# MPI-SWS/RedQueen

Measured on AMD Instinct MI355X. Metric: redqueen_replicas_per_sec, higher is better.
Workload: dtype f64; 1 GPU; C3 syn1k: 1000 followers, 50 sources (25 Poisson2 rate 1 + 25 Hawkes l0=1 a=1 b=10), degree 5, T=100, q=1e6, s=1, RedQueen, randomized worlds; replicas_per_gpu=10000, global_batch=10000, parallelism=replica-sharded dp1, replicas_per_chunk=10000

## Files before the change

redqueen_amd/csrc/rq_api.cpp:

```cpp
#include <hip/hip_runtime.h>

#include <algorithm>
#include <cstring>
#include <memory>
#include <mutex>
#include <new>
#include <vector>

#include "../../include/rq.h"
#include "rq_internal.h"

using rqh::align_up;
using rqh::CtrlTables;
using rqh::GraphTopo;
using rqh::Knobs;
using rqh::Plan;

namespace {

template <class T>
struct DevBuf {
    T* p = nullptr;
    size_t n = 0;
    ~DevBuf() { if (p) (void)hipFree(p); }
// ... 537 lines not shown

int rq_graph_source_ids(rq_graph_t g, int64_t* ids)
{
    if (!g || !ids) return RQ_EINVAL;
    std::copy(g->src_id.begin(), g->src_id.end(), ids);
    return RQ_OK;
}

int rq_graph_followers(rq_graph_t g, int64_t* ids)
{
    if (!g || !ids) return RQ_EINVAL;
    std::copy(g->fol_ids.begin(), g->fol_ids.end(), ids);
    return RQ_OK;
}

int rq_workspace_size(rq_graph_t g, const rq_batch_desc* b, size_t* bytes)
{
    if (!bytes) return RQ_EINVAL;
    Plan p;
    const int rc = plan_call(g, b, rqh::read_knobs(), 0.0, &p);
    if (rc) return rc;
    *bytes = p.total;
    return RQ_OK;
}

int rq_plan_info(rq_graph_t g, const rq_batch_desc* b, int64_t* info)
{
    return rq_plan_info_n(g, b, info, 8);
}

int rq_plan_info_n(rq_graph_t g, const rq_batch_desc* b, int64_t* out, int n)
{
    if (!out || n < 0) return RQ_EINVAL;
    int64_t info[9];
    Plan p;
    const int rc = plan_call(g, b, rqh::read_knobs(), 0.0, &p);
    if (rc) return rc;
    rqh::plan_info(p, b->ctrl_kind, info);
    std::copy(info, info + std::min(n, 9), out);
    return RQ_OK;
}

int rq_event_capacity(rq_graph_t g, const rq_batch_desc* b, int64_t* cap)
{
    if (!cap) return RQ_EINVAL;
    Plan p;
    const int rc = plan_call(g, b, rqh::read_knobs(), 0.0, &p);
    if (rc) return rc;
    *cap = p.cap_rows;
    return RQ_OK;
}

int rq_run_batch(rq_graph_t g, const rq_batch_desc* b, const rq_outputs* out, void* workspace,
                 size_t workspace_bytes, void* hip_stream)
{
    const Knobs kn = rqh::read_knobs();
    Plan p;
    int rc = plan_call(g, b, kn, (double)workspace_bytes, &p);
    if (rc) return rc;
    if (!out || !out->metrics || !out->counts || !out->status || !workspace) return RQ_EINVAL;
    if (workspace_bytes < p.total) return RQ_EINVAL;
    if ((b->flags & RQ_RUN_EVENT_LOG) && (!out->ev_t || !out->ev_src || out->ev_cap < 1))
        return RQ_EINVAL;
    char* ws = (char*)workspace;
    hipStream_t pst[3] = {(hipStream_t)hip_stream, nullptr, nullptr};

    if ((rc = stage_tables(g, p, b, rqh::ctrl_tables(*g, b), ws, pst[0]))) return rc;
    if (hipMemsetAsync(out->status, 0, sizeof(int32_t) * p.R, pst[0]) != hipSuccess) return RQ_EHIP;
    Join join{pst, t_pipes.of(pst[0])};
    if ((rc = fork_streams(p.nbuf, &join))) return rc;

    int64_t ci = 0;
// ... 501 lines not shown
```

redqueen_amd/csrc/rq_device.h:

```cpp
#pragma once
#include <hip/hip_runtime.h>
#include <stdint.h>

#include "rq_spec.h"

#pragma clang fp contract(off)

#define RQ_INF __builtin_huge_val()

namespace rq {

static __constant__ uint64_t rq_exp_tab_c[RQ_EXP_TAB_N] = RQ_EXP_TAB_INIT;

__device__ __forceinline__ void philox4x32_10(uint32_t c[4], uint32_t k0, uint32_t k1)
{
#pragma unroll
    for (int r = 0; r < 10; ++r) {
        const uint64_t p0 = (uint64_t)0xD2511F53u * c[0];
        const uint64_t p1 = (uint64_t)0xCD9E8D57u * c[2];
        const uint32_t n0 = (uint32_t)(p1 >> 32) ^ c[1] ^ k0;
        const uint32_t n2 = (uint32_t)(p0 >> 32) ^ c[3] ^ k1;
        c[0] = n0;
        c[1] = (uint32_t)p1;
        c[2] = n2;
// ... 44 lines not shown
}

__device__ __forceinline__ double wave_min(double v)
{
#pragma unroll
    for (int o = 32; o > 0; o >>= 1) v = fmin(v, __shfl_xor(v, o, 64));
    return v;
}

__device__ __forceinline__ double bcast_d(double v, int src_lane)
{
    const uint64_t b = rq_dbl_bits(v);
    const uint32_t lo = (uint32_t)__builtin_amdgcn_readlane((int)(uint32_t)b, src_lane);
    const uint32_t hi = (uint32_t)__builtin_amdgcn_readlane((int)(uint32_t)(b >> 32), src_lane);
    return rq_bits_dbl(((uint64_t)hi << 32) | lo);
}

__device__ __forceinline__ int bcast_i(int v, int src_lane)
{
    return __builtin_amdgcn_readlane(v, src_lane);
}

__device__ __forceinline__ uint64_t sgpr_u64(uint64_t v)
{
    const uint32_t lo = (uint32_t)__builtin_amdgcn_readfirstlane((int)(uint32_t)v);
    const uint32_t hi = (uint32_t)__builtin_amdgcn_readfirstlane((int)(uint32_t)(v >> 32));
    return ((uint64_t)hi << 32) | lo;
}
__device__ __forceinline__ int64_t bcast_i64(int64_t v, int src_lane)
{
    const uint32_t lo = (uint32_t)__builtin_amdgcn_readlane((int)(uint32_t)v, src_lane);
    const uint32_t hi = (uint32_t)__builtin_amdgcn_readlane((int)(uint32_t)((uint64_t)v >> 32), src_lane);
    return (int64_t)(((uint64_t)hi << 32) | lo);
}

__device__ __forceinline__ void wave_lds_sync()
{
    __builtin_amdgcn_fence(__ATOMIC_RELEASE, "wavefront");
    __builtin_amdgcn_wave_barrier();
    __builtin_amdgcn_fence(__ATOMIC_ACQUIRE, "wavefront");
}
__device__ __forceinline__ void wave_mem_sync()
{
    __builtin_amdgcn_fence(__ATOMIC_RELEASE, "workgroup");
    __builtin_amdgcn_wave_barrier();
    __builtin_amdgcn_fence(__ATOMIC_ACQUIRE, "workgroup");
}

__device__ __forceinline__ int popc(uint64_t m) { return __popcll(m); }

template <int CTRL, int ROWMASK>
__device__ __forceinline__ uint32_t dpp_u32(uint32_t v)
{
    return (uint32_t)__builtin_amdgcn_update_dpp((int)0xFFFFFFFF, (int)v, CTRL, ROWMASK, 0xF, false);
}
__device__ __forceinline__ uint32_t umin32(uint32_t a, uint32_t b) { return a < b ? a : b; }

__device__ __forceinline__ uint32_t wave_min_u32(uint32_t v)
{
    v = umin32(v, dpp_u32<0xB1, 0xF>(v));
    v = umin32(v, dpp_u32<0x4E, 0xF>(v));
    v = umin32(v, dpp_u32<0x141, 0xF>(v));
    v = umin32(v, dpp_u32<0x140, 0xF>(v));
    v = umin32(v, dpp_u32<0x142, 0xA>(v));
    v = umin32(v, dpp_u32<0x143, 0xC>(v));
    return (uint32_t)__builtin_amdgcn_readlane((int)v, 63);
// ... 87 lines not shown
        v |= dpp0<0x111, 0xF>(v) & c0;
        v |= dpp0<0x112, 0xF>(v) & c1;
        v |= dpp0<0x114, 0xF>(v) & c2;
        v |= dpp0<0x118, 0xF>(v) & c3;
        v |= dpp0<0x142, 0xA>(v) & c4;
        v |= dpp0<0x143, 0xC>(v) & c5;
        return v;
    }
    __device__ __forceinline__ uint32_t scan_or_z(uint32_t m) const
    {
        uint32_t t = dppz<0x111>(m);
        uint32_t v = m | (t & c0);
        t = dppz<0x112>(v);
        v |= t & c1;
        t = dppz<0x114>(v);
        v |= t & c2;
        t = dppz<0x118>(v);
        v |= t & c3;
        t = (uint32_t)__builtin_amdgcn_update_dpp((int)t, (int)v, 0x142, 0xA, 0xF, false);
        v |= t & c4;
        t = (uint32_t)__builtin_amdgcn_update_dpp((int)t, (int)v, 0x143, 0xC, 0xF, false);
        v |= t & c5;
        return v;
    }
    __device__ __forceinline__ uint32_t scan_add(uint32_t v) const
    {
        v += dpp0<0x111, 0xF>(v) & c0;
        v += dpp0<0x112, 0xF>(v) & c1;
        v += dpp0<0x114, 0xF>(v) & c2;
        v += dpp0<0x118, 0xF>(v) & c3;
        v += dpp0<0x142, 0xA>(v) & c4;
        v += dpp0<0x143, 0xC>(v) & c5;
        return v;
    }
};

__device__ __forceinline__ int stage_rank(const double* st_t, int n, double ti, int lane)
{
    int rnk = 0;
    for (int q = 0; q < n; q += 8) {
        double2 x[4];
#pragma unroll
        for (int u = 0; u < 4; ++u) x[u] = *reinterpret_cast<const double2*>(st_t + q + 2 * u);
#pragma unroll
        for (int u = 0; u < 4; ++u) rnk += (x[u].x < ti ? 1 : 0) + (x[u].y < ti ? 1 : 0);
    }
    const uint32_t sum = wave_sum_u32(lane < n ? (uint32_t)rnk : 0u);
    if (sum == (uint32_t)(n * (n - 1) / 2)) return rnk;
    rnk = 0;
    for (int q = 0; q < n; q += 2) {
        const double2 x = *reinterpret_cast<const double2*>(st_t + q);
        rnk += (x.x < ti || (x.x == ti && q < lane)) ? 1 : 0;
        rnk += (x.y < ti || (x.y == ti && q + 1 < lane)) ? 1 : 0;
    }
    return rnk;
}

__device__ __forceinline__ double min_raw(double a, double b)
{
    double r;
    __asm__("v_min_f64 %0, %1, %2\n\ts_nop 1" : "=v"(r) : "v"(a), "v"(b));
    return r;
}

__device__ __forceinline__ double wave_min_f64(double x)
{
// ... 340 lines not shown
```

redqueen_amd/csrc/rq_host.h:

```cpp
#pragma once
#include <stddef.h>
#include <stdint.h>

#include <vector>

#include "../../include/rq.h"

#define RQ_MAX_STREAMS 2048
#define RQ_NPSUM1_LDS 516
#ifndef RQ_MRG_LB
#define RQ_MRG_LB 1024
#endif
#define RQ_MG_B 512
#define RQ_MAX_STREAMS_MRG (RQ_MG_B * RQ_MG_B)

struct SweepInst {
    bool fused;
    int nK;
    bool col16;
    bool log;
    bool gs;
    bool bits;
    bool bl;
    bool mrg;
    int spl;
    int W;
    bool gt;
    bool pw;
    bool pair;
    bool scan;
};
#define RQ_FWS_NL 66
#define RQ_FWS_LDS_BYTES(nK) ((size_t)8 * (((nK) + 2 + 3) * RQ_FWS_NL + 4))

#ifndef RQ_FOLLOWERS_TILE_SINKS
#define RQ_FOLLOWERS_TILE_SINKS 2048
#endif
static_assert(RQ_FOLLOWERS_TILE_SINKS >= 1 &&
                  (long long)RQ_FOLLOWERS_TILE_SINKS * (12 + 8 * (RQ_MAX_K + 2) + 8) <= 160 * 1024,
              "a tile of every nK / rows variant must fit one workgroup's LDS");

int rq_sweep_blocks_per_cu(const SweepInst& i, int wpb, size_t lds);
int rq_fw_blocks_per_cu(const SweepInst& i, int wpb, size_t lds);
int rq_cu_count();

namespace rqh {

inline size_t align_up(size_t x, size_t a) { return (x + a - 1) / a * a; }

inline int followers_tiles(int n_sinks) { return (n_sinks + RQ_FOLLOWERS_TILE_SINKS - 1) / RQ_FOLLOWERS_TILE_SINKS; }
inline size_t followers_tiled_ws_bytes(int n_sinks, int64_t n_rep)
{
    return align_up((size_t)4 * (size_t)n_rep * (size_t)followers_tiles(n_sinks), 256);
}

template <class T>
struct Knob {
    bool set = false;
    T v{};
};
struct Knobs {
    Knob<double> ws_budget_gb;
    double cap_squeeze = 1.0;
    Knob<int> mg_grp;
    bool mrg = true;
    Knob<int> g_collds;
    int g_w = 0;
    bool skip = true;
    bool fwm = true;
    bool ctrl_draws = true;
    bool sweep_scan = true;
    int fw_w = 0;
    int pipe = 2;
    Knob<int64_t> pipe_chunk;
    bool order = false;

    int sweep_dbg = 0;
    double fw_tile = 58.0;
    Knob<int> fw_hmin, fw_thr, fw_hfill;
    int fw_static = 0;
    bool clk_merge = false;

    Knob<int> rp_chunk;
    bool rp_small = true;
    bool clk_replay = false;
};
Knobs read_knobs();

struct GraphTopo {
    int n_str = 0, ctrl_idx = -1, n_sinks = 0, n_fol = 0;
    int64_t n_edges = 0, ctrl_src_id = 0;
    double start = 0.0, end = 0.0;
    std::vector<int64_t> src_id;
    std::vector<int> kind, orig_idx, arr_off, arr_n;
    std::vector<int> is_static;
    std::vector<uint32_t> seed;
    std::vector<double> p0, p1, p2, arr_a, arr_b;
    std::vector<int> csr_ptr, csr_col, outdeg_f, fol;
    std::vector<int64_t> fol_ids;
    std::vector<int64_t> sink_ids;
    std::vector<int> csr_col_el;
    std::vector<int> col_to_fol;
    bool multi = false, ctrl_dup = false;
    bool rd_ties = false, rd_ties_ctrl = false;
// ... 5 lines not shown
    int n_tiles = 0;
    std::vector<int> tile_ptr, tile_col;
    int ctrl_arr_off = 0, ctrl_arr_n = 0;
};
int topo_build(const rq_graph_desc* d, GraphTopo* g);

struct Plan {
    int nK = 1, spl = 1, wpb = 4, n_sinks_pad = 0;
    int64_t R = 0, chunk = 0, capsum = 0, cap_rows = 0;
    int64_t rep_lo = 0, rep_cnt = 0;
    std::vector<int> cap;
    std::vector<int64_t> st_off;
    std::vector<int> rd_k;
    bool log = false, bits = false;
    bool bl = false;
    size_t g_fb = 0, g_etab = 0, g_inv = 0, g_skip = 0;
    bool g_inv_sh = false;
    bool gs = false;
    int64_t gs_slots = 0, gs_stride = 0;
    bool fw = false;
    int fw_h = 8, mstride = 1;
    bool mrg = false;
    bool lmrg = false;
    bool gt = false;
    size_t off_mt = 0, off_mj = 0, off_mjh = 0, off_mlen = 0;
    int64_t mrg_stride = 0;
    int n_grp = 1;
    int grp_sz = RQ_MG_B;
    int64_t sub_stride = 0;
    size_t off_sub_t = 0, off_sub_j = 0, off_sub_len = 0;
    bool fwm = false;
    bool pair = false;
    bool scan = false;
    int gwpb = 4, gwin = 16, gcol_lds = 1, gcol16 = 0;
    size_t g_col = 0, g_ptr = 0, g_odf = 0, g_cbf = 0, g_wave = 0, g_wave_stride = 0, g_rank_off = 0,
           g_win_off = 0, g_x_off = 0, g_total = 0, g_stage_off = 0;
    size_t tables_bytes = 0;
    int wpc = 0;
    int nbuf = 1;
    bool order = false;
    size_t off_set0 = 0, set_stride = 0, off_ord = 0;
    size_t off_pwc = 0, off_pwmax = 0;
    size_t off_invc = 0, off_streams = 0, off_slen = 0, off_rt = 0, off_rs = 0, off_rv = 0,
           off_rc = 0, off_sall = 0, off_wq = 0, off_stoff = 0, off_cap = 0, off_rdk = 0, off_repidx = 0, off_gs = 0,
           total = 0;
};

int make_plan(const GraphTopo& g, const rq_batch_desc* b, const Knobs& kn, double budget, Plan* p);
SweepInst sweep_inst(const Plan& p, int ctrl_kind);
void plan_info(const Plan& p, int ctrl_kind, int64_t info[9]);

struct CtrlTables {
    std::vector<double> invc;
    std::vector<double> pwc, pwmax;
};
CtrlTables ctrl_tables(const GraphTopo& g, const rq_batch_desc* b);

}
```

redqueen_amd/csrc/rq_plan.cpp:

```cpp
#include <algorithm>
#include <cmath>
#include <cstdlib>

#include "rq_host.h"
#include "rq_tables.h"

namespace rqh {

Knobs read_knobs()
{
    Knobs k;
    if (const char* e = getenv("RQ_WS_BUDGET_GB")) k.ws_budget_gb = {true, atof(e)};
    if (const char* e = getenv("RQ_CAP_SQUEEZE")) k.cap_squeeze = std::max(0.01, std::min(1.0, atof(e)));
    if (const char* e = getenv("RQ_MG_GRP")) k.mg_grp = {true, atoi(e)};
    if (const char* e = getenv("RQ_MRG")) k.mrg = atoi(e) != 0;
    if (const char* e = getenv("RQ_G_COLLDS")) k.g_collds = {true, atoi(e)};
    if (const char* e = getenv("RQ_G_W")) k.g_w = atoi(e);
    if (const char* e = getenv("RQ_SKIP")) k.skip = atoi(e) != 0;
    if (const char* e = getenv("RQ_FWM")) k.fwm = atoi(e) != 0;
    if (const char* e = getenv("RQ_CTRL_DRAWS")) k.ctrl_draws = atoi(e) != 0;
    if (const char* e = getenv("RQ_SWEEP_SCAN")) k.sweep_scan = atoi(e) != 0;
    if (const char* e = getenv("RQ_FW_W")) k.fw_w = atoi(e);
    if (const char* e = getenv("RQ_PIPE")) k.pipe = std::max(1, std::min(3, atoi(e)));
    if (const char* e = getenv("RQ_PIPE_CHUNK")) k.pipe_chunk = {true, std::max<int64_t>(64, atoll(e))};
    if (const char* e = getenv("RQ_ORDER")) k.order = atoi(e) != 0;
    if (const char* e = getenv("RQ_SWEEP_DBG")) k.sweep_dbg = atoi(e);
    if (const char* e = getenv("RQ_FW_TILE")) k.fw_tile = atof(e);
    if (const char* e = getenv("RQ_FW_HMIN")) k.fw_hmin = {true, atoi(e)};
    if (const char* e = getenv("RQ_FW_THR")) k.fw_thr = {true, atoi(e)};
    if (const char* e = getenv("RQ_FW_HFILL")) k.fw_hfill = {true, atoi(e)};
    static const int fw_static = getenv("RQ_FW_STATIC") ? atoi(getenv("RQ_FW_STATIC")) : 0;
    k.fw_static = fw_static;
    k.clk_merge = getenv("RQ_CLK_MERGE") != nullptr;
    if (const char* e = getenv("RQ_RP_CHUNK")) k.rp_chunk = {true, atoi(e)};
    if (const char* e = getenv("RQ_RP_SMALL")) k.rp_small = atoi(e) != 0;
    k.clk_replay = getenv("RQ_CLK_REPLAY") != nullptr;
    return k;
}

namespace {

constexpr size_t kLdsMax = 160 * 1024;

double stream_mean_var(const GraphTopo* g, int j, int kind, const rq_batch_desc* b, double* var)
{
    const double span = g->end - g->start;
    double m = 0.0;
    *var = 0.0;
    switch (kind) {
    case RQ_SRC_POISSON:
    case RQ_SRC_POISSON2: {
        const double rate = j == g->ctrl_idx ? b->ctrl_rate_max : g->p0[j];
        m = std::max(0.0, rate) * span;
        *var = m;
// ... 18 lines not shown
            const double hi = std::min(k + 1 < n ? g->arr_a[off + k + 1] : g->end, g->end);
            if (hi > lo) m += std::max(0.0, g->arr_b[off + k]) * (hi - lo);
        }
        *var = m;
        break;
    }
    case RQ_SRC_REALDATA:
        m = g->arr_n[j];
        *var = 0.0;
        break;
    default:
        break;
    }
    return m;
}

SweepInst sweep_inst(const Plan& p, int ctrl_kind, bool fused, int W, bool col16, bool gs, bool gt)
{
    SweepInst i{};
    i.fused = fused;
    i.nK = p.nK;
    i.col16 = col16;
    i.log = p.log;
    i.gs = gs;
    i.bits = p.bits;
    i.bl = p.bl;
    i.mrg = fused ? p.fwm : p.mrg;
    i.spl = p.spl;
    i.W = W;
    i.gt = gt;
    i.pw = ctrl_kind == RQ_SRC_OPTPW;
    i.pair = fused && i.mrg && p.pair;
    i.scan = fused && i.mrg && p.scan;
    return i;
}
int sweep_blocks_per_cu(const SweepInst& i, int wpb, size_t lds)
{
    return i.fused ? rq_fw_blocks_per_cu(i, wpb, lds) : rq_sweep_blocks_per_cu(i, wpb, lds);
}

void plan_layout(const GraphTopo* g, const rq_batch_desc* b, Plan* p);

int plan_args(const GraphTopo* g, const rq_batch_desc* b, Plan* p)
{
    if (!b) return RQ_EINVAL;
    if (b->nK < 1 || b->nK > RQ_MAX_K || !b->Ks) return RQ_EINVAL;
    if (b->n_grid < 1 || b->n_rep < 1) return RQ_EINVAL;
    const int ck = b->ctrl_kind;
    if (ck != RQ_SRC_OPT && ck != RQ_SRC_OPTPW && ck != RQ_SRC_POISSON2 && ck != RQ_SRC_PWCONST &&
        ck != RQ_SRC_REALDATA && ck != RQ_SRC_NONE)
        return RQ_EINVAL;
    if (ck == RQ_SRC_OPT && (!b->q || (g->n_fol > 0 && !b->s))) return RQ_EINVAL;
    if (ck == RQ_SRC_OPTPW &&
        (!b->q || b->n_seg < 1 || b->n_seg > 4096 || !(b->period > 0.0) || (g->n_fol > 0 && !b->s_pw)))
        return RQ_EINVAL;
    if (ck == RQ_SRC_POISSON2 && !b->ctrl_rate) return RQ_EINVAL;
    if ((ck == RQ_SRC_PWCONST) && g->ctrl_arr_n < 1) return RQ_EINVAL;
    p->nK = b->nK;
    if (b->rep_cnt < 0 || (b->rep_cnt > 0 && (b->rep_lo < 0 || b->rep_lo + b->rep_cnt > b->n_rep)))
        return RQ_EINVAL;
    p->rep_lo = b->rep_cnt > 0 ? b->rep_lo : 0;
    p->rep_cnt = b->rep_cnt > 0 ? b->rep_cnt : b->n_rep;
    const int64_t Rall = (int64_t)b->n_grid * p->rep_cnt;
    if (b->replica0 < 0 || b->n_local < 0 || b->replica0 + b->n_local > Rall) return RQ_EINVAL;
    p->R = b->n_local > 0 ? b->n_local : Rall - b->replica0;
    if (p->R < 1) return RQ_EINVAL;
// ... 148 lines not shown
                }
            }
        }
    }
    if (best < 0) return false;
    p->g_skip = 0;
    if (p->bl && p->mrg && !p->gs) {
        const size_t st2 = align_up(p->g_wave_stride + 8 * (size_t)g->n_str, 16);
        const size_t tot2 = p->g_wave + p->gwpb * st2;
        const SweepInst inst = sweep_inst(*p, b->ctrl_kind, false, p->gwin, p->gcol16, p->gs, p->gt);
        int blocks = tot2 <= kLdsMax ? sweep_blocks_per_cu(inst, p->gwpb, tot2) : 0;
        if (tot2 <= kLdsMax && blocks <= 0) blocks = (int)std::min<size_t>(kLdsMax / tot2, 16 / p->gwpb);
        const bool on = blocks * p->gwpb >= p->wpc && kn.skip;
        if (on) {
            p->g_skip = p->g_wave_stride;
            p->g_wave_stride = st2;
            p->g_total = tot2;
        }
    }
    return true;
}

void plan_fused_lds(const GraphTopo* g, const rq_batch_desc* b, const Knobs& kn, Plan* p)
{
    const bool pw = b->ctrl_kind == RQ_SRC_OPTPW;
    p->fw = !p->log && !p->bl && g->n_str <= 64 && b->sweep_mode != 4 && b->sweep_mode != 5 &&
            b->sweep_mode != 6;
    p->fwm = p->fw && !pw && b->sweep_mode != 7;
    p->fwm = p->fwm && kn.fwm;
    p->pair = p->fwm && b->ctrl_kind == RQ_SRC_OPT;
    p->pair = p->pair && kn.ctrl_draws;
    p->scan = p->fwm && !(b->flags & RQ_RUN_EVENT_LOG) && b->max_events < 0;
    p->scan = p->scan && kn.sweep_scan;
    if (p->fw) {
        int best = -1;
        const int c16 = p->bits ? 1 : (g->n_sinks <= 65535 ? 1 : 0);
        if (pw && !c16) p->fw = false;
        const size_t colb = p->bits ? 4 * (size_t)(g->n_str + 1) * p->mstride
                                    : (c16 ? 2 * g->csr_col.size() : 0);
        size_t sh = 0;
        const size_t o_col = sh;  sh = align_up(sh + colb, 16);
        const size_t o_ptr = sh;  sh = align_up(sh + 4 * (g->n_str + 1), 16);
        const size_t o_odf = sh;  sh = align_up(sh + 4 * g->n_str, 16);
        const size_t o_cbf = sh;  sh = align_up(sh + 4 * g->n_str, 16);
        const size_t o_etab = sh; sh = align_up(sh + RQ_EXP_TAB_N * 8, 16);
        const int only_w = kn.fw_w;
        for (int W : {32, 16, 8}) {
            if (!p->fw) break;
            if (only_w && W != only_w) continue;
            if (pw && W != 16) continue;
            if (W == 32 && !p->bits) continue;
            const int H = W > 16 ? 8 : W / 2;
            const size_t r_off = align_up(8 * (size_t)g->n_str, 16);
            const size_t w_off = align_up(r_off + (p->bits ? 8 * (size_t)((g->nw + 1) & ~1) : 2 * (size_t)p->n_sinks_pad), 16);
            const size_t s_off = align_up(w_off + (p->fwm ? 0 : 8 * (size_t)g->n_str * (W + 1)), 16);
            size_t stride = align_up(s_off + 64 * 12, 16);
            if (p->scan) stride = std::max(stride, align_up(RQ_FWS_LDS_BYTES(p->nK), 16));
            for (int wpb : {16, 12, 10, 8, 6, 5, 4, 3, 2, 1}) {
                const size_t tot = sh + wpb * stride;
                if (tot > kLdsMax) continue;
                int blocks = sweep_blocks_per_cu(sweep_inst(*p, b->ctrl_kind, true, W, c16, false, false), wpb, tot);
                if (blocks <= 0) blocks = (int)std::min<size_t>(kLdsMax / tot, 16 / wpb);
                const int waves = blocks * wpb;
                const int score = waves * 4 + (W == 16 ? 2 : W == 32 ? 1 : 0);
                if (score > best) {
                    best = score;
                    p->wpc = waves;
                    p->gwin = W; p->fw_h = H; p->gwpb = wpb; p->gcol_lds = c16; p->gcol16 = c16;
                    p->g_col = o_col; p->g_ptr = o_ptr; p->g_odf = o_odf; p->g_cbf = o_cbf;
                    p->g_wave = sh; p->g_wave_stride = stride; p->g_rank_off = r_off;
                    p->g_win_off = w_off; p->g_stage_off = s_off; p->g_x_off = 0; p->g_total = tot;
                    p->g_etab = o_etab;
                }
            }
        }
        if (best < 0) p->fw = false;
    }
    if (!p->fw) p->fwm = false;
    if (!p->fwm) p->pair = p->scan = false;
    if (p->fw) p->mrg = p->fwm;
}

}

SweepInst sweep_inst(const Plan& p, int ctrl_kind)
{
    return sweep_inst(p, ctrl_kind, p.fw, p.gwin, p.gcol16, p.gs, p.gt);
}

void plan_info(const Plan& p, int ctrl_kind, int64_t info[9])
{
    info[0] = (p.log ? (p.gs ? 4 : 1) : (p.bits ? 2 : (p.bl ? 3 : 0))) + (p.fwm ? 20 : p.fw ? 10 : 0);
    info[1] = p.mrg ? 0 : p.spl;
    info[2] = p.gwin;
    info[3] = p.gwpb;
    info[4] = sweep_blocks_per_cu(sweep_inst(p, ctrl_kind), p.gwpb, p.g_total);
    info[5] = p.gcol_lds;
    info[6] = (int64_t)p.g_total;
    info[7] = p.chunk;
    info[8] = p.scan ? 1 : 0;
}

int make_plan(const GraphTopo& topo, const rq_batch_desc* b, const Knobs& kn, double budget, Plan* p)
{
    const GraphTopo* g = &topo;
    if (const int rc = plan_args(g, b, p)) return rc;
    if (const int rc = plan_capacities(g, b, kn, p)) return rc;
    const int ck = b->ctrl_kind;
    if (g->ctrl_dup && (ck == RQ_SRC_OPT || ck == RQ_SRC_OPTPW)) return RQ_EINVAL;
    if (g->n_str > RQ_MAX_STREAMS_MRG) return RQ_EUNSUPPORTED;
    p->spl = g->n_str <= 64 ? 1 : g->n_str <= 128 ? 2 : g->n_str <= 256 ? 4 : 8;
    p->n_sinks_pad = (g->n_sinks + 1) | 1;
// ... 122 lines not shown
```

redqueen_amd/csrc/rq_sweep_fw.hip:

```cpp
#include <hip/hip_runtime.h>
#include <stdint.h>

#include "rq_device.h"
#include "rq_internal.h"
#include "rq_sweep_core.h"
#include "rq_gen.h"
#include "rq_scan_rows.h"
#include <type_traits>
#include <cstdlib>

#pragma clang fp contract(off)

using namespace rq;

constexpr int fws_tu(int nk) { return nk == 1 ? 4 : 2; }
template <int NK>
__device__ __forceinline__ void fw_scan_rows(int64_t n, double S, double end, const double* Rt, const double* Rs,
                                             const uint32_t* Rv, const uint32_t* Rc, double* lds, double* out)
{
    constexpr int NV = NK + 2;
    static_assert(RQ_FWS_LDS_BYTES(NK) == 8 * (size_t)npsum_lds_doubles<NV, RQ_FWS_NL>(), "the planner's size");
    const int lane = lane_id();
    if (n == 0) {
        if (lane < NV) out[lane] = __builtin_nan("");
        return;
    }
    __asm__ volatile("s_waitcnt vmcnt(0)" ::: "memory");
    __builtin_amdgcn_fence(__ATOMIC_RELEASE, "workgroup");
    __builtin_amdgcn_fence(__ATOMIC_ACQUIRE, "workgroup");
    double res[NV];
    scan_rows<NK, fws_tu(NK), RQ_FWS_NL>(n, S, end, Rt, Rs, Rv, Rc, lds, res);
    if (lane == 0) {
#pragma unroll
        for (int s = 0; s < NV; ++s) out[s] = res[s];
    }
}
template <int NK, class COL, int W, int H, bool BITS, bool PW, bool MRG, bool PAIR = false, bool SCAN = false>
__device__ __forceinline__ void sweep_fw_body(SweepArgs a)
{
    static_assert((W & (W - 1)) == 0 && H <= W, "ring");
    static_assert(!SCAN || MRG, "the sweep's own scan: merged instances only");
    extern __shared__ double lds_g[];
    char* base = reinterpret_cast<char*>(lds_g);
    const int lane = lane_id();
    const int w = threadIdx.x >> 6;
    int* cptr = reinterpret_cast<int*>(base + a.lds_ptr);
    int* odf = reinterpret_cast<int*>(base + a.lds_odf);
    int* cbf = reinterpret_cast<int*>(base + a.lds_cbf);
    constexpr bool col_lds = sizeof(COL) == 2;
    COL* col_l = reinterpret_cast<COL*>(base + a.lds_col);
    const int* col_g = a.csr_col;
    if (col_lds && !BITS)
        for (int e = threadIdx.x; e < a.n_csr; e += blockDim.x) col_l[e] = (COL)a.csr_col[e];
    uint32_t* msk = reinterpret_cast<uint32_t*>(base + a.lds_mask);
    const int ms = a.mstride;
    if (BITS)
        for (int e = threadIdx.x; e < (a.n_str + 1) * ms; e += blockDim.x) {
            const int jj = e / ms, ww = e - jj * ms;
            msk[e] = (jj < a.n_str && ww < a.nw) ? a.masks[jj * a.nw + ww] : 0u;
        }
    uint64_t* etab = reinterpret_cast<uint64_t*>(base + a.lds_etab);
    for (int e = threadIdx.x; e < RQ_EXP_TAB_N; e += blockDim.x) etab[e] = rq_exp_tab_c[e];
    for (int j = threadIdx.x; j <= a.n_str; j += blockDim.x) cptr[j] = a.csr_ptr[j];
    for (int j = threadIdx.x; j < a.n_str; j += blockDim.x) {
        odf[j] = a.outdeg_f[j];
        cbf[j] = a.cbf_g[j];
    }
    __syncthreads();
    char* wb = base + a.lds_wave + (size_t)w * a.lds_wave_stride;
    double* invc = reinterpret_cast<double*>(wb);
    int16_t* rank = reinterpret_cast<int16_t*>(wb + a.lds_rank_off);
    uint2* ft = reinterpret_cast<uint2*>(wb + a.lds_rank_off);
    double* ring = reinterpret_cast<double*>(wb + a.lds_win_off) + lane * (W + 1);
    double* st_t = reinterpret_cast<double*>(wb + a.lds_stage_off);
// ... 28 lines not shown
    if (lane < a.n_str && !MRG) gen.init(a.gen, lane, i, etab);
    else gen.none();
    int pos = 0, fil = 0;
    const int64_t mb = MRG ? rl * a.mrg_stride : 0;
    auto mload = [&](int64_t e, double& t_, int& j_) __attribute__((always_inline)) {
        int64_t x = mb;
        __asm__ volatile("" : "+v"(x));
        t_ = a.mrg_t[x + e];
        j_ = a.mrg_j[x + e];
    };
    const int mlen = MRG ? a.mrg_len[rl] : 0;
    int mpos = 0;
    double nxt_t = RQ_INF;
    int nxt_j = 0;
    if (MRG && lane < mlen) mload(lane, nxt_t, nxt_j);

    const bool opt = a.ctrl_kind == RQ_SRC_OPT || a.ctrl_kind == RQ_SRC_OPTPW;
    const double* pwc = PW ? a.pw_c + (size_t)g * a.n_str * a.n_seg : nullptr;
    const double* pwm = PW ? a.pw_max + (size_t)g * a.n_str : nullptr;
    double opt_next = opt ? a.start : RQ_INF;
    const int64_t k = a.seed_mod > 0 ? i % a.seed_mod : i;
    const uint32_t oseed = a.ctrl_seed ? a.ctrl_seed[i] : a.ctrl_seed0 + (uint32_t)k;
    uint64_t ndraw = 0;
    double px0 = 0.0, px1 = 0.0;
    auto colat = [&](int e) -> int { return col_lds ? (int)col_l[e] : col_g[e]; };
    const int fol0 = cptr[a.ctrl_idx];
    auto folat = [&](int f) -> int { return colat(fol0 + f); };

    Agg<NK> ag;
    ag.init(a.Ks);
    AggB agb;
    if (BITS) {
        agb.init(msk, a.nw, ms, a.ctrl_idx, lane);
        if (lane < ((a.nw + 1) & ~1)) ft[lane] = make_uint2(agb.F, 0u);
    }
    RowStage<NK> rs;
    const int64_t rbase = rl * a.cap_rows;
    rs.init(a.rows_t, a.rows_sum, a.rows_valid, a.rows_cnt, rbase, a.cap_rows);

    int64_t n_events = 0, posts = 0, world = 0;
    int status = 0;
    double span = -1.0;
    bool stop = false;
    const int thr = a.fw_thr;
    auto refill_pass = [&]() __attribute__((always_inline)) {
#ifdef RQ_PHASE_CLOCK
        ck[6] += 1;
        ck[7] += __popcll(__ballot(!gen.done && fil - pos < W));
#endif
        if (!gen.done && fil - pos < W) {
            double tv;
            if (gen.step(&tv, a.end)) {
                ring[fil & (W - 1)] = tv;
                ++fil;
            }
        }
    };
    for (;;) {
        int n = 0;
        bool act, fin;
        double tt, tx = 0.0;
        int tj;
        if constexpr (MRG) {
            if (mpos >= mlen) break;
            n = mlen - mpos < 64 ? mlen - mpos : 64;
            act = lane < n;
            tt = act ? nxt_t : RQ_INF;
// ... 140 lines not shown
        const bool has_o = own_b && a.n_fol > 0;
        const bool has_w = act && e1 > e0;
        int64_t osum = 0, wsum = 0;
        int oval = 0, wval = 0;
        int ocnt[NK], wcnt[NK];
#pragma unroll
        for (int kq = 0; kq < NK; ++kq) ocnt[kq] = wcnt[kq] = 0;
        if (a.dbg == 1) {
        } else if (BITS) {
            const bool rst = own_b || strm_own;
            const uint64_t rm = __ballot(rst);
            const bool hasr = mbcnt64_incl(rm) != 0;
            const bool wl = act && !strm_own;
            const int deg = wl ? e1 - e0 : 0;
            const int odv = wl ? od : 0;
            SegFlags sf;
            sf.init(rst);
            const int pdeg = (int)wave_scan_add((uint32_t)deg);
            const int64_t sfq = (int64_t)(int)sf.scan_add((uint32_t)odv) + (hasr ? 0 : agb.sumF);
            int64_t dec = 0;
            for (uint64_t b = rm; b; b &= b - 1) {
                const int r = __ffsll((unsigned long long)b) - 1;
                const int64_t D = r == 0 ? agb.sumF : bcast_i64(sfq, r - 1);
                if (lane >= r) dec += D;
            }
            wsum = agb.sumR + pdeg - dec;
            osum = agb.sumR + (pdeg - deg) - dec;
            const bool vfull = agb.nvalid == a.n_sinks;
            const int last = n - 1;
            const uint32_t* mr = msk + (wl ? tj : a.n_str) * ms;
            const bool wlast = lane == last;
            int cw = 0, vw = 0, vo = 0;
            uint32_t nV = agb.V;
            if (vfull) {
                for (int ww = 0; ww < a.nw; ww += 2) {
                    const uint2 f0 = ft[ww], f1 = ft[ww + 1];
                    const uint32_t u0 = sf.scan_or_z(mr[ww]);
                    const uint32_t u1 = sf.scan_or_z(mr[ww + 1]);
                    const uint32_t t0 = (hasr ? f0.x : f0.y) & ~u0;
                    const uint32_t t1 = (hasr ? f1.x : f1.y) & ~u1;
                    cw += __popc(t0) + __popc(t1);
                    if (wlast) {
                        ft[ww].y = t0;
                        ft[ww + 1].y = t1;
                    }
                }
            } else {
                for (int ww = 0; ww < a.nw; ++ww) {
                    const uint2 fw2 = ft[ww];
                    const uint32_t m = mr[ww];
                    const uint32_t u = sf.scan_or_z(m);
                    const uint32_t tq = (hasr ? fw2.x : fw2.y) & ~u;
                    cw += __popc(tq);
                    if (wlast) ft[ww].y = tq;
                    const uint32_t Vw = (uint32_t)__builtin_amdgcn_readlane((int)agb.V, ww);
                    const uint32_t x = wave_scan_or(m);
                    const uint32_t vq = Vw | x | (hasr ? fw2.x : 0u);
                    vw += __popc(vq);
                    const uint32_t xe = (uint32_t)__builtin_amdgcn_update_dpp(0, (int)x, 0x138, 0xF, 0xF, false);
                    vo += __popc(Vw | xe | fw2.x);
                    nV = (uint32_t)wlane((int)nV, __builtin_amdgcn_readlane((int)vq, last), ww);
                }
            }
            wcnt[0] = cw;
            ocnt[0] = a.n_fol;
            wval = vfull ? a.n_sinks : vw;
            oval = vfull ? a.n_sinks : vo;
// ... 86 lines not shown
    if (BITS) {
        agb.sync();
        ag.nvalid = agb.nvalid;
    }
    if (lane == 0) {
        int64_t* cnto = a.counts + o * 4;
        cnto[0] = posts;
        cnto[1] = world;
        cnto[2] = n_events;
        cnto[3] = rs.nrow;
        a.sall[rl] = ag.nvalid;
        if (rs.nrow == 0) status |= RQ_ST_EMPTY;
        if (status) atomicOr(&a.status[o], status);
    }
    if constexpr (SCAN)
        fw_scan_rows<NK>(rs.nrow, (double)ag.nvalid, a.end, a.rows_t + rbase, a.rows_sum + rbase,
                         a.rows_valid + rbase, a.rows_cnt + rbase * NK, reinterpret_cast<double*>(wb),
                         a.metrics + o * (NK + 2));
    if (!a.wq) break;
    int nx = 0;
    if (lane == 0) nx = atomicAdd(a.wq, 1);
    qi = nslot + __builtin_amdgcn_readfirstlane(nx);
    }
}

template <int NK, class COL, int W, int H, bool BITS, bool PW = false, bool MRG = false>
__global__ __launch_bounds__(1024) void rq_sweep_fw(SweepArgs a)
{
    sweep_fw_body<NK, COL, W, H, BITS, PW, MRG>(a);
}
#ifndef RQ_FWM_WPE
#define RQ_FWM_WPE 4
#endif
template <int NK, class COL, bool BITS, bool PAIR = false, bool SCAN = false>
__global__ __launch_bounds__(1024) __attribute__((amdgpu_waves_per_eu(RQ_FWM_WPE))) void rq_sweep_fwm(SweepArgs a)
{
    sweep_fw_body<NK, COL, 16, 8, BITS, false, true, PAIR, SCAN>(a);
}

template <class COL, int W, bool PW = false>
static SweepKernel fw_nk(int nK)
{
    constexpr int H = W > 16 ? 8 : W / 2;
    switch (nK) {
    case 1: return rq_sweep_fw<1, COL, W, H, false, PW>;
    case 2: return rq_sweep_fw<2, COL, W, H, false, PW>;
    case 3: return rq_sweep_fw<3, COL, W, H, false, PW>;
    default: return rq_sweep_fw<4, COL, W, H, false, PW>;
    }
}
template <class COL, bool PAIR, bool SCAN>
static SweepKernel fwm_nk(int nK)
{
    switch (nK) {
    case 1: return rq_sweep_fwm<1, COL, false, PAIR, SCAN>;
    case 2: return rq_sweep_fwm<2, COL, false, PAIR, SCAN>;
    case 3: return rq_sweep_fwm<3, COL, false, PAIR, SCAN>;
    default: return rq_sweep_fwm<4, COL, false, PAIR, SCAN>;
    }
}
template <bool PAIR, bool SCAN>
static SweepKernel fwm_kernel(const SweepInst& i)
{
    if (i.bits) return rq_sweep_fwm<1, uint16_t, true, PAIR, SCAN>;
    return i.col16 ? fwm_nk<uint16_t, PAIR, SCAN>(i.nK) : fwm_nk<int, PAIR, SCAN>(i.nK);
}
static SweepKernel fw_kernel(const SweepInst& i)
{
    if (i.mrg) {
        if (i.pw) return nullptr;
        if (i.pair)
            return i.scan ? fwm_kernel<true, true>(i) : fwm_kernel<true, false>(i);
        return i.scan ? fwm_kernel<false, true>(i) : fwm_kernel<false, false>(i);
    }
    if (i.pair || i.scan) return nullptr;
    if (i.pw) {
        if (!i.col16 || i.W != 16) return nullptr;
        return i.bits ? rq_sweep_fw<1, uint16_t, 16, 8, true, true> : fw_nk<uint16_t, 16, true>(i.nK);
    }
    if (i.bits)
        return i.W == 32 ? rq_sweep_fw<1, uint16_t, 32, 8, true>
             : i.W == 16 ? rq_sweep_fw<1, uint16_t, 16, 8, true> : rq_sweep_fw<1, uint16_t, 8, 4, true>;
    if (i.W == 16) return i.col16 ? fw_nk<uint16_t, 16>(i.nK) : fw_nk<int, 16>(i.nK);
    return i.col16 ? fw_nk<uint16_t, 8>(i.nK) : fw_nk<int, 8>(i.nK);
}

static int occ_fw_t(SweepKernel k, int wpb, size_t lds)
{
    return rq_occupancy(k, 64 * wpb, lds);
}
static hipError_t launch_fw_t(SweepKernel k, const SweepArgs& a, hipStream_t s)
{
    unsigned blocks = (unsigned)((a.n_chunk + a.wpb - 1) / a.wpb);
    if (a.wq) {
        const int nb = occ_fw_t(k, a.wpb, a.lds_total);
        const unsigned cap = (unsigned)(nb > 0 ? nb : 1) * (unsigned)rq_cu_count();
        if (cap < blocks) blocks = cap;
    }
    hipLaunchKernelGGL(k, dim3(blocks), dim3(64 * a.wpb), a.lds_total, s, a);
    return hipGetLastError();
}

hipError_t rq_launch_sweep_fw(const SweepArgs& a, const SweepInst& i, hipStream_t s)
{
    if (a.n_chunk <= 0) return hipSuccess;
    if (i.pair && a.ctrl_kind != RQ_SRC_OPT) return hipErrorInvalidValue;
    if (i.scan && (!a.metrics || a.ev_t || a.max_events >= 0 || a.lds_wave_stride < RQ_FWS_LDS_BYTES(i.nK)))
        return hipErrorInvalidValue;
    const SweepKernel k = fw_kernel(i);
    return k ? launch_fw_t(k, a, s) : hipErrorInvalidValue;
}

int rq_fw_blocks_per_cu(const SweepInst& i, int wpb, size_t lds)
{
    const SweepKernel k = fw_kernel(i);
    return k ? occ_fw_t(k, wpb, lds) : -1;
}
```

redqueen_amd/engine.py:

```python
import ctypes as C
import math

import numpy as np
import torch

from . import _lib as L

KIND_BY_NAME = {"Poisson": L.SRC_POISSON, "Poisson2": L.SRC_POISSON2, "Hawkes": L.SRC_HAWKES,
                "PiecewiseConst": L.SRC_PWCONST, "RealData": L.SRC_REALDATA, "Opt": L.SRC_OPT}
CTRL_BY_NAME = {"opt": L.SRC_OPT, "poisson": L.SRC_POISSON2, "pwconst": L.SRC_PWCONST,
                "times": L.SRC_REALDATA, "wall": L.SRC_NONE, "sig": L.SRC_OPTPW}


def _arr(x, dt):
    return np.ascontiguousarray(np.asarray(x, dtype=dt))


def _source_class(name):
    if isinstance(name, str):
        if name in KIND_BY_NAME:
            return None
        from .opt_model import SimOpts
        cls = SimOpts.broadcasters.get(name)
        if cls is None:
# ... 229 lines not shown
        elif self.plugins and (randomize or rd_override is not None):
            self._plugin_streams(b, keep, dev, R_all, gids, world_seed, int(seed_mod), rd_override)
        if ck == L.SRC_POISSON2:
            if ctrl_rate is None:
                raise ValueError("ctrl_rate required for a Poisson controlled source")
            cr = torch.as_tensor(ctrl_rate, dtype=torch.float64, device=dev).reshape(-1)
            if cr.numel() == 1:
                cr = cr.expand(R_all)
            cr = cr.contiguous()
            keep.append(cr)
            b.ctrl_rate = cr.data_ptr()
            b.ctrl_rate_max = float(cr.max().item()) if cr.numel() else 0.0
        b.Ks = Ks.ctypes.data_as(L._pi32)
        b.nK = Ks.size
        b.max_events = -1 if max_events is None or max_events == float("inf") else int(max_events)
        b.flags = L.RUN_EVENT_LOG if event_log else 0
        b.cap_scale = float(cap_scale)
        b.chunk = int(chunk)
        b.sweep_mode = int(sweep_mode)
        b.replica0 = int(replica0)
        b.n_local = int(n_local)
        b.rep_lo = lo
        b.rep_cnt = int(rep_cnt)
        if rep_idx is not None:
            keep.append(gids)
            b.rep_idx = gids.ctypes.data_as(L._pi64)
        if spw is not None:
            b.n_seg = spw.shape[2]
            b.period = float(period)
            b.s_pw = spw.ctypes.data_as(L._pd)
        lib = L.lib()
        if plan_only:
            b.ws_budget = self._ws_budget(dev)
            info = (C.c_int64 * 9)()
            L.check("rq_plan_info_n", lib.rq_plan_info_n(self._h, C.byref(b), info, 9))
            keys = ("variant", "sources_per_lane", "ring_depth", "waves_per_block",
                    "blocks_per_cu", "columns_in_lds", "lds_bytes_per_block", "chunk", "sweep_scan")
            return dict(zip(keys, (int(v) for v in info)))
        return self._run_loop(lib, b, keep, dev, R, Ks, n_grid, n_rep, ck, event_log,
                              gids, check, stream)

    def _launch(self, lib, b, dev, R, Ks, n_grid, n_rep, event_log, use):
        sk = use.cuda_stream
        metrics = torch.empty((R, Ks.size + 2), dtype=torch.float64, device=dev)
        counts = torch.empty((R, 4), dtype=torch.int64, device=dev)
        status = torch.empty(R, dtype=torch.int32, device=dev)
        out = L.Outputs()
        out.metrics, out.counts, out.status = metrics.data_ptr(), counts.data_ptr(), status.data_ptr()
        ev_t = ev_src = None
        if event_log:
            cap = C.c_int64()
            L.check("rq_event_capacity", lib.rq_event_capacity(self._h, C.byref(b), C.byref(cap)))
            ev_t = torch.empty((R, cap.value), dtype=torch.float64, device=dev)
            ev_src = torch.empty((R, cap.value), dtype=torch.int32, device=dev)
            out.ev_t, out.ev_src, out.ev_cap = ev_t.data_ptr(), ev_src.data_ptr(), cap.value
        nbytes = C.c_size_t()
        b.ws_budget = self._ws_budget(dev, sk)
        L.check("rq_workspace_size", lib.rq_workspace_size(self._h, C.byref(b), C.byref(nbytes)))
        ws = self._wss.get(sk)
        if ws is None or ws.numel() < nbytes.value:
            self._wss[sk] = ws = None
            ws = self._wss[sk] = torch.empty(max(256, nbytes.value), dtype=torch.uint8, device=dev)
        L.check("rq_run_batch", lib.rq_run_batch(self._h, C.byref(b), C.byref(out),
                                                 ws.data_ptr(), ws.numel(), sk))
        return BatchResult(self, metrics, counts, status, ev_t, ev_src, Ks, n_grid, int(n_rep))

    CAP_MEMO_SHARE = 1.0 / 16

    def _cap_key(self, b, ck):
        qk = None
# ... 528 lines not shown
```

Before: 4.428 million replicas/s.

## Add event-blocked phase C in merged sink-bit sweep with column-blocked mask layout

Adds a BLK variant of the merged sink-bit follower sweep. It lays the sink-bit masks out in column blocks so each 16-lane group handles four events across a slice of sink words, and chains the OR-scans with DPP carries instead of a per-word wave scan. Per-event counts are then gathered with permlane swaps and a bpermute. The aim is to cut the serial per-word scan loop over nw words in the full-event phase, at the cost of a larger mask stride in LDS, which can reduce occupancy. It is enabled by default when nw is at least 13 (1000 followers gives about 32 words).

```diff
diff --git a/redqueen_amd/csrc/rq_api.cpp b/redqueen_amd/csrc/rq_api.cpp
--- a/redqueen_amd/csrc/rq_api.cpp
+++ b/redqueen_amd/csrc/rq_api.cpp
@@ -593,12 +593,13 @@
 int rq_plan_info_n(rq_graph_t g, const rq_batch_desc* b, int64_t* out, int n)
 {
     if (!out || n < 0) return RQ_EINVAL;
-    int64_t info[9];
+    int64_t info[10];
     Plan p;
     const int rc = plan_call(g, b, rqh::read_knobs(), 0.0, &p);
     if (rc) return rc;
     rqh::plan_info(p, b->ctrl_kind, info);
-    std::copy(info, info + std::min(n, 9), out);
+    info[9] = p.blk ? 1 : 0;
+    std::copy(info, info + std::min(n, 10), out);
     return RQ_OK;
 }
 
diff --git a/redqueen_amd/csrc/rq_device.h b/redqueen_amd/csrc/rq_device.h
--- a/redqueen_amd/csrc/rq_device.h
+++ b/redqueen_amd/csrc/rq_device.h
@@ -100,6 +100,15 @@
     const uint32_t lo = (uint32_t)__builtin_amdgcn_readlane((int)(uint32_t)v, src_lane);
     const uint32_t hi = (uint32_t)__builtin_amdgcn_readlane((int)(uint32_t)((uint64_t)v >> 32), src_lane);
     return (int64_t)(((uint64_t)hi << 32) | lo);
+}
+
+template <class T>
+__device__ __forceinline__ T* lds_opaque(T* p)
+{
+    typedef __attribute__((address_space(3))) char* lds_ptr;
+    uint32_t a = (uint32_t)(size_t)(lds_ptr)(char*)p;
+    __asm__("" : "+v"(a));
+    return (T*)(char*)(lds_ptr)(size_t)a;
 }
 
 __device__ __forceinline__ void wave_lds_sync()
@@ -253,6 +262,48 @@
         v += dpp0<0x142, 0xA>(v) & c4;
         v += dpp0<0x143, 0xC>(v) & c5;
         return v;
+    }
+};
+
+struct BlkFlags {
+    uint32_t c0, c1, c2, c3;
+    uint32_t d0, d1, d2, d3;
+    uint32_t kc;
+    __device__ __forceinline__ void init(uint64_t rm, int lane)
+    {
+        const int g = lane & 15;
+        const uint32_t h = (uint32_t)(rm >> (4 * g)) & 0xFu;
+        c0 = (h & 1u) - 1u;
+        c1 = ((h >> 1) & 1u) - 1u;
+        c2 = ((h >> 2) & 1u) - 1u;
+        c3 = (h >> 3) - 1u;
+        uint32_t f = h ? 1u : 0u;
+        d0 = f - 1u;  f |= dpp0<0x111, 0xF>(f);
+        d1 = f - 1u;  f |= dpp0<0x112, 0xF>(f);
+        d2 = f - 1u;  f |= dpp0<0x114, 0xF>(f);
+        d3 = f - 1u;
+        kc = g == 0 ? c0 : 0u;
+        __asm__("" : "+v"(c0), "+v"(c1), "+v"(c2), "+v"(c3), "+v"(d0), "+v"(d1), "+v"(d2), "+v"(d3), "+v"(kc));
+    }
+    __device__ __forceinline__ void chain(uint32_t p, uint32_t m0, uint32_t m1, uint32_t m2, uint32_t m3, uint32_t& u0,
+                                          uint32_t& u1, uint32_t& u2, uint32_t& u3) const
+    {
+        u0 = m0 | (p & c0);
+        u1 = m1 | (u0 & c1);
+        u2 = m2 | (u1 & c2);
+        u3 = m3 | (u2 & c3);
+    }
+    __device__ __forceinline__ uint32_t carry(uint32_t t) const
+    {
+        uint32_t s = dppz<0x111>(t);
+        uint32_t v = t | (s & d0);
+        s = dppz<0x112>(v);
+        v |= s & d1;
+        s = dppz<0x114>(v);
+        v |= s & d2;
+        s = dppz<0x118>(v);
+        v |= s & d3;
+        return dppz<0x111>(v);
     }
 };
 
diff --git a/redqueen_amd/csrc/rq_host.h b/redqueen_amd/csrc/rq_host.h
--- a/redqueen_amd/csrc/rq_host.h
+++ b/redqueen_amd/csrc/rq_host.h
@@ -29,7 +29,11 @@
     bool pw;
     bool pair;
     bool scan;
+    bool blk;
 };
+#define RQ_BLK_CB(nw) ((((nw) + 7) >> 3) << 1)
+#define RQ_BLK_MSTRIDE(nw) (4 * RQ_BLK_CB(nw) + 4)
+#define RQ_BLK_MIN_NW 13
 #define RQ_FWS_NL 66
 #define RQ_FWS_LDS_BYTES(nK) ((size_t)8 * (((nK) + 2 + 3) * RQ_FWS_NL + 4))
 
@@ -70,6 +74,7 @@
     bool fwm = true;
     bool ctrl_draws = true;
     bool sweep_scan = true;
+    bool phasec_blk = true;
     int fw_w = 0;
     int pipe = 2;
     Knob<int64_t> pipe_chunk;
@@ -141,6 +146,7 @@
     bool fwm = false;
     bool pair = false;
     bool scan = false;
+    bool blk = false;
     int gwpb = 4, gwin = 16, gcol_lds = 1, gcol16 = 0;
     size_t g_col = 0, g_ptr = 0, g_odf = 0, g_cbf = 0, g_wave = 0, g_wave_stride = 0, g_rank_off = 0,
            g_win_off = 0, g_x_off = 0, g_total = 0, g_stage_off = 0;
diff --git a/redqueen_amd/csrc/rq_plan.cpp b/redqueen_amd/csrc/rq_plan.cpp
--- a/redqueen_amd/csrc/rq_plan.cpp
+++ b/redqueen_amd/csrc/rq_plan.cpp
@@ -20,6 +20,7 @@
     if (const char* e = getenv("RQ_FWM")) k.fwm = atoi(e) != 0;
     if (const char* e = getenv("RQ_CTRL_DRAWS")) k.ctrl_draws = atoi(e) != 0;
     if (const char* e = getenv("RQ_SWEEP_SCAN")) k.sweep_scan = atoi(e) != 0;
+    if (const char* e = getenv("RQ_PHASEC_BLK")) k.phasec_blk = atoi(e) != 0;
     if (const char* e = getenv("RQ_FW_W")) k.fw_w = atoi(e);
     if (const char* e = getenv("RQ_PIPE")) k.pipe = std::max(1, std::min(3, atoi(e)));
     if (const char* e = getenv("RQ_PIPE_CHUNK")) k.pipe_chunk = {true, std::max<int64_t>(64, atoll(e))};
@@ -104,6 +105,7 @@
     i.pw = ctrl_kind == RQ_SRC_OPTPW;
     i.pair = fused && i.mrg && p.pair;
     i.scan = fused && i.mrg && p.scan;
+    i.blk = fused && i.mrg && p.blk;
     return i;
 }
 int sweep_blocks_per_cu(const SweepInst& i, int wpb, size_t lds)
@@ -318,11 +320,14 @@
     p->pair = p->pair && kn.ctrl_draws;
     p->scan = p->fwm && !(b->flags & RQ_RUN_EVENT_LOG) && b->max_events < 0;
     p->scan = p->scan && kn.sweep_scan;
+    p->blk = p->fwm && p->bits && g->nw >= RQ_BLK_MIN_NW;
+    p->blk = p->blk && kn.phasec_blk;
+    const int mstride = p->blk ? RQ_BLK_MSTRIDE(g->nw) : p->mstride;
     if (p->fw) {
         int best = -1;
         const int c16 = p->bits ? 1 : (g->n_sinks <= 65535 ? 1 : 0);
         if (pw && !c16) p->fw = false;
-        const size_t colb = p->bits ? 4 * (size_t)(g->n_str + 1) * p->mstride
+        const size_t colb = p->bits ? 4 * (size_t)(g->n_str + 1) * mstride
                                     : (c16 ? 2 * g->csr_col.size() : 0);
         size_t sh = 0;
         const size_t o_col = sh;  sh = align_up(sh + colb, 16);
@@ -338,7 +343,8 @@
             if (W == 32 && !p->bits) continue;
             const int H = W > 16 ? 8 : W / 2;
             const size_t r_off = align_up(8 * (size_t)g->n_str, 16);
-            const size_t w_off = align_up(r_off + (p->bits ? 8 * (size_t)((g->nw + 1) & ~1) : 2 * (size_t)p->n_sinks_pad), 16);
+            const size_t ftw = p->blk ? 4 * (size_t)RQ_BLK_CB(g->nw) : (size_t)((g->nw + 1) & ~1);
+            const size_t w_off = align_up(r_off + (p->bits ? 8 * ftw : 2 * (size_t)p->n_sinks_pad), 16);
             const size_t s_off = align_up(w_off + (p->fwm ? 0 : 8 * (size_t)g->n_str * (W + 1)), 16);
             size_t stride = align_up(s_off + 64 * 12, 16);
             if (p->scan) stride = std::max(stride, align_up(RQ_FWS_LDS_BYTES(p->nK), 16));
@@ -363,7 +369,8 @@
         if (best < 0) p->fw = false;
     }
     if (!p->fw) p->fwm = false;
-    if (!p->fwm) p->pair = p->scan = false;
+    if (!p->fwm) p->pair = p->scan = p->blk = false;
+    if (p->blk) p->mstride = mstride;
     if (p->fw) p->mrg = p->fwm;
 }
 
diff --git a/redqueen_amd/csrc/rq_sweep_fw.hip b/redqueen_amd/csrc/rq_sweep_fw.hip
--- a/redqueen_amd/csrc/rq_sweep_fw.hip
+++ b/redqueen_amd/csrc/rq_sweep_fw.hip
@@ -35,11 +35,13 @@
         for (int s = 0; s < NV; ++s) out[s] = res[s];
     }
 }
-template <int NK, class COL, int W, int H, bool BITS, bool PW, bool MRG, bool PAIR = false, bool SCAN = false>
+template <int NK, class COL, int W, int H, bool BITS, bool PW, bool MRG, bool PAIR = false, bool SCAN = false,
+          bool BLK = false>
 __device__ __forceinline__ void sweep_fw_body(SweepArgs a)
 {
     static_assert((W & (W - 1)) == 0 && H <= W, "ring");
     static_assert(!SCAN || MRG, "the sweep's own scan: merged instances only");
+    static_assert(!BLK || (MRG && BITS), "event-blocked phase C: the merged sink-bit instances only");
     extern __shared__ double lds_g[];
     char* base = reinterpret_cast<char*>(lds_g);
     const int lane = lane_id();
@@ -134,7 +136,7 @@
     AggB agb;
     if (BITS) {
         agb.init(msk, a.nw, ms, a.ctrl_idx, lane);
-        if (lane < ((a.nw + 1) & ~1)) ft[lane] = make_uint2(agb.F, 0u);
+        if (lane < (BLK ? 4 * RQ_BLK_CB(a.nw) : (a.nw + 1) & ~1)) ft[lane] = make_uint2(agb.F, 0u);
     }
     RowStage<NK> rs;
     const int64_t rbase = rl * a.cap_rows;
@@ -341,7 +343,53 @@
             const bool wlast = lane == last;
             int cw = 0, vw = 0, vo = 0;
             uint32_t nV = agb.V;
-            if (vfull) {
+            if (BLK && vfull) {
+                const int CB = RQ_BLK_CB(a.nw);
+                int ln = lane;
+                __asm__ volatile("" : "+v"(ln));
+                int* st_r = reinterpret_cast<int*>(wb + a.lds_stage_off);
+                st_r[ln] = (wl ? tj : a.n_str) * ms;
+                wave_lds_sync();
+                const int g4 = ln & 15, cb0 = (ln >> 4) * CB;
+                const int4 ro = *reinterpret_cast<const int4*>(st_r + 4 * g4);
+                BlkFlags bf;
+                bf.init(rm, ln);
+                auto m0 = lds_opaque(reinterpret_cast<const uint2*>(msk + ro.x + cb0));
+                auto m1 = lds_opaque(reinterpret_cast<const uint2*>(msk + ro.y + cb0));
+                auto m2 = lds_opaque(reinterpret_cast<const uint2*>(msk + ro.z + cb0));
+                auto m3 = lds_opaque(reinterpret_cast<const uint2*>(msk + ro.w + cb0));
+                auto fb = lds_opaque(reinterpret_cast<uint4*>(ft + cb0));
+                const bool wgrp = g4 == (last >> 2);
+                uint32_t q0 = 0, q1 = 0, q2 = 0, q3 = 0;
+                auto column = [&](uint2 f, uint32_t w0, uint32_t w1, uint32_t w2, uint32_t w3)
+                                  __attribute__((always_inline)) -> uint32_t {
+                    w0 |= (f.x & ~f.y) & bf.kc;
+                    uint32_t l0, l1, l2, l3, u0, u1, u2, u3;
+                    bf.chain(0u, w0, w1, w2, w3, l0, l1, l2, l3);
+                    bf.chain(bf.carry(l3), w0, w1, w2, w3, u0, u1, u2, u3);
+                    q0 += __popc(f.x & ~u0);
+                    q1 += __popc(f.x & ~u1);
+                    q2 += __popc(f.x & ~u2);
+                    const uint32_t t3 = f.x & ~u3;
+                    q3 += __popc(t3);
+                    return t3;
+                };
+                for (int c = 0; c < CB; c += 2, ++fb, ++m0, ++m1, ++m2, ++m3) {
+                    const uint4 f = *fb;
+                    const uint2 w0 = *m0, w1 = *m1, w2 = *m2, w3 = *m3;
+                    const uint32_t ta = column(make_uint2(f.x, f.y), w0.x, w1.x, w2.x, w3.x);
+                    const uint32_t tb = column(make_uint2(f.z, f.w), w0.y, w1.y, w2.y, w3.y);
+                    if (wgrp) {
+                        fb->y = ta;
+                        fb->w = tb;
+                    }
+                }
+                const auto s01 = __builtin_amdgcn_permlane32_swap(q0, q1, false, false);
+                const auto s23 = __builtin_amdgcn_permlane32_swap(q2, q3, false, false);
+                const auto s4 = __builtin_amdgcn_permlane16_swap(s01[0] + s01[1], s23[0] + s23[1], false, false);
+                const int src = (((ln & 1) << 1 | ((ln >> 1) & 1)) << 4) | (ln >> 2);
+                cw = __builtin_amdgcn_ds_bpermute(src << 2, (int)(s4[0] + s4[1]));
+            } else if (vfull) {
                 for (int ww = 0; ww < a.nw; ww += 2) {
                     const uint2 f0 = ft[ww], f1 = ft[ww + 1];
                     const uint32_t u0 = sf.scan_or_z(mr[ww]);
@@ -494,10 +542,10 @@
 #ifndef RQ_FWM_WPE
 #define RQ_FWM_WPE 4
 #endif
-template <int NK, class COL, bool BITS, bool PAIR = false, bool SCAN = false>
+template <int NK, class COL, bool BITS, bool PAIR = false, bool SCAN = false, bool BLK = false>
 __global__ __launch_bounds__(1024) __attribute__((amdgpu_waves_per_eu(RQ_FWM_WPE))) void rq_sweep_fwm(SweepArgs a)
 {
-    sweep_fw_body<NK, COL, 16, 8, BITS, false, true, PAIR, SCAN>(a);
+    sweep_fw_body<NK, COL, 16, 8, BITS, false, true, PAIR, SCAN, BLK>(a);
 }
 
 template <class COL, int W, bool PW = false>
@@ -524,7 +572,9 @@
 template <bool PAIR, bool SCAN>
 static SweepKernel fwm_kernel(const SweepInst& i)
 {
-    if (i.bits) return rq_sweep_fwm<1, uint16_t, true, PAIR, SCAN>;
+    if (i.blk && !i.bits) return nullptr;
+    if (i.bits)
+        return i.blk ? rq_sweep_fwm<1, uint16_t, true, PAIR, SCAN, true> : rq_sweep_fwm<1, uint16_t, true, PAIR, SCAN>;
     return i.col16 ? fwm_nk<uint16_t, PAIR, SCAN>(i.nK) : fwm_nk<int, PAIR, SCAN>(i.nK);
 }
 static SweepKernel fw_kernel(const SweepInst& i)
@@ -535,7 +585,7 @@
             return i.scan ? fwm_kernel<true, true>(i) : fwm_kernel<true, false>(i);
         return i.scan ? fwm_kernel<false, true>(i) : fwm_kernel<false, false>(i);
     }
-    if (i.pair || i.scan) return nullptr;
+    if (i.pair || i.scan || i.blk) return nullptr;
     if (i.pw) {
         if (!i.col16 || i.W != 16) return nullptr;
         return i.bits ? rq_sweep_fw<1, uint16_t, 16, 8, true, true> : fw_nk<uint16_t, 16, true>(i.nK);
@@ -569,6 +619,7 @@
     if (i.pair && a.ctrl_kind != RQ_SRC_OPT) return hipErrorInvalidValue;
     if (i.scan && (!a.metrics || a.ev_t || a.max_events >= 0 || a.lds_wave_stride < RQ_FWS_LDS_BYTES(i.nK)))
         return hipErrorInvalidValue;
+    if (i.blk && a.mstride != RQ_BLK_MSTRIDE(a.nw)) return hipErrorInvalidValue;
     const SweepKernel k = fw_kernel(i);
     return k ? launch_fw_t(k, a, s) : hipErrorInvalidValue;
 }
diff --git a/redqueen_amd/engine.py b/redqueen_amd/engine.py
--- a/redqueen_amd/engine.py
+++ b/redqueen_amd/engine.py
@@ -285,10 +285,11 @@
         lib = L.lib()
         if plan_only:
             b.ws_budget = self._ws_budget(dev)
-            info = (C.c_int64 * 9)()
-            L.check("rq_plan_info_n", lib.rq_plan_info_n(self._h, C.byref(b), info, 9))
+            info = (C.c_int64 * 10)()
+            L.check("rq_plan_info_n", lib.rq_plan_info_n(self._h, C.byref(b), info, 10))
             keys = ("variant", "sources_per_lane", "ring_depth", "waves_per_block",
-                    "blocks_per_cu", "columns_in_lds", "lds_bytes_per_block", "chunk", "sweep_scan")
+                    "blocks_per_cu", "columns_in_lds", "lds_bytes_per_block", "chunk", "sweep_scan",
+                    "sweep_blk")
             return dict(zip(keys, (int(v) for v in info)))
         return self._run_loop(lib, b, keep, dev, R, Ks, n_grid, n_rep, ck, event_log,
                               gids, check, stream)
```

Measured after the change: 4.584 million replicas/s (median of 6 runs). 3.5% higher.
